# toposware/certificate-stark

Measured on AMD Instinct MI355X. Metric: proofs/sec, state_transition AIR @ 2^20 steps (complete prove(): trace gen, LDE, Blake3 commitments, constraint evaluation, composition, DEEP, FRI, 96 queries), higher is better.
Workload: dtype u64 (63-bit prime field, Montgomery) + u32 (Blake3)

## Files before the change

certificate-stark_amd/csrc/capi.hip:

```cpp
#include <hip/hip_runtime.h>
#include <stdio.h>
#include <stdlib.h>
#include <string.h>
#include <deque>
#include <new>
#include <vector>
#include "../../include/cstark.h"
#include "air_tx_host.h"
#include "blake3.h"
#include "ctx.h"
#include "constraints.h"
#include "deep.h"
#include "ext.h"
#include "generator_fold.h"
#include "hostfield.h"
#include "ntt.h"
#include "trace_gen.h"

namespace cs { thread_local char g_err[512] = ""; }
using cs::fail;
using cs::NttPlan;
using cs::CosetTable;
using cs::PeriodicTable;
using cs::g_err;
// ... 581 lines not shown
    HIP_TRY(hipSetDevice(c->device));
    const size_t N = (size_t)1 << (log_n + log_blowup);
    RC_TRY(ensure_ws(c, 2 * N * 8));
    uint64_t *nat = (uint64_t *)c->ws, *h = nat + N;
    if (log_blowup <= 3) {
        const NttPlan *pn, *pN;
        RC_TRY(get_plan(c, log_n, &pn));
        RC_TRY(get_plan(c, log_n + log_blowup, &pN));
        cs::NttArgs a{};
        a.in = d_combined; a.scratch = h; a.out = nat; a.width = 1u << log_blowup; a.batch = 1; a.log_n = log_n;
        a.w = pn->winv; a.post_scale = pn->n_inv; a.do_scale = true; a.inverse = true; a.aux = pn->aux_winv;
        HIP_TRY(cs::ntt_columns(a, c->stream));
        const uint64_t b_inv = cs::host::inv(cs::host::from_u64(1ull << log_blowup));
        HIP_TRY(cs::coset_combine(nat, h, log_n, log_blowup, pN->winv, b_inv, c->stream));
        HIP_TRY(cs::split_columns(h, d_cols, log_n, log_blowup, cs::host::inv(cs::host::lde_offset()), c->stream));
        return CSTARK_OK;
    }
    HIP_TRY(cs::interleave_cosets(d_combined, nat, log_n, log_blowup, c->stream));
    const NttPlan *p;
    RC_TRY(get_plan(c, log_n + log_blowup, &p));
    cs::NttArgs a{};
    a.in = nat; a.scratch = nat; a.out = h; a.width = 1; a.batch = 1; a.log_n = log_n + log_blowup;
    a.w = p->winv; a.post_scale = p->n_inv; a.do_scale = true; a.inverse = true; a.aux = p->aux_winv;
    HIP_TRY(cs::ntt_columns(a, c->stream));
    HIP_TRY(cs::split_columns(h, d_cols, log_n, log_blowup, cs::host::inv(cs::host::lde_offset()), c->stream));
    return CSTARK_OK;
}

int cstark_evaluate_polys_at(cstark_ctx *c, const uint64_t *d_coeffs, uint32_t width, uint32_t log_n, const uint64_t *points, uint32_t npts,
                             uint64_t *out ) {
    if (!c || !d_coeffs || !points || !out || width == 0 || npts == 0 || npts > 16) return fail(CSTARK_ERR_INVALID_ARG, "cstark_evaluate_polys_at: bad argument");
    if (log_n > 30) return fail(CSTARK_ERR_INVALID_ARG, "bad polynomial size");
    HIP_TRY(hipSetDevice(c->device));
    const size_t need = ((size_t)npts + (size_t)npts * width + cs::poly_eval_scratch_words(width, log_n, npts)) * 8;
    if (need > c->desc_bytes) {
        if (c->desc_buf) { HIP_TRY(hipStreamSynchronize(c->stream)); HIP_TRY(hipFree(c->desc_buf)); c->desc_buf = nullptr; c->desc_bytes = 0; }
        HIP_TRY(hipMalloc(&c->desc_buf, need));
        c->desc_bytes = need;
    }
    uint64_t *d_pts = (uint64_t *)c->desc_buf, *d_out = d_pts + npts, *d_scr = d_out + (size_t)npts * width;
    HIP_TRY(hipMemcpyAsync(d_pts, points, (size_t)npts * 8, hipMemcpyHostToDevice, c->stream));
    HIP_TRY(cs::poly_eval(d_coeffs, width, log_n, d_pts, npts, d_out, d_scr, c->stream));
    HIP_TRY(hipMemcpyAsync(out, d_out, (size_t)npts * width * 8, hipMemcpyDeviceToHost, c->stream));
    HIP_TRY(cs::stream_wait(c->stream));
    return CSTARK_OK;
}

int cstark_deep_composition(cstark_ctx *c, const uint64_t *d_trace_lde, const uint64_t *d_comp_lde, uint32_t width, uint32_t n_comp,
                            uint64_t z, const uint64_t *ood_trace, const uint64_t *ood_comp, const uint64_t *alpha, const uint64_t *beta,
                            const uint64_t *delta, uint64_t deg_a, uint64_t deg_b, uint64_t *d_out, uint32_t log_n, uint32_t log_blowup,
                            uint32_t k0, uint32_t nk) {
    if (!c || !d_trace_lde || !d_comp_lde || !ood_trace || !ood_comp || !alpha || !beta || !delta || !d_out || nk == 0 || width == 0 || n_comp == 0)
        return fail(CSTARK_ERR_INVALID_ARG, "cstark_deep_composition: bad argument");
    if (log_n < cs::NTT_MIN_LOG_N || log_n > cs::NTT_MAX_LOG_N || log_blowup > 6 || (uint64_t)k0 + nk > (1ull << log_blowup)) return fail(CSTARK_ERR_INVALID_ARG, "bad domain parameters");
    HIP_TRY(hipSetDevice(c->device));
    const NttPlan *plan;
    RC_TRY(get_plan(c, log_n, &plan));
    const size_t b = (size_t)1 << log_blowup, nco = 2 * (size_t)width + n_comp, words = 2 * nco + b;
    if (c->deep_words < words) {
        HIP_TRY(hipStreamSynchronize(c->stream));
        if (c->deep_buf) { HIP_TRY(hipFree(c->deep_buf)); c->deep_buf = nullptr; }
        if (c->deep_stage) { HIP_TRY(hipHostFree(c->deep_stage)); c->deep_stage = nullptr; }
        c->deep_words = 0;
        HIP_TRY(hipMalloc((void **)&c->deep_buf, words * 8));
        HIP_TRY(hipHostMalloc((void **)&c->deep_stage, words * 8, hipHostMallocDefault));
        if (!c->deep_ev) HIP_TRY(hipEventCreateWithFlags(&c->deep_ev, hipEventDisableTiming));
        c->deep_words = words;
    } else {
        HIP_TRY(hipEventSynchronize(c->deep_ev));
    }
    uint64_t *blk = c->deep_stage;
    memcpy(blk, alpha, width * 8); memcpy(blk + width, beta, width * 8); memcpy(blk + 2 * width, delta, n_comp * 8);
    memcpy(blk + nco, ood_trace, 2 * (size_t)width * 8); memcpy(blk + nco + 2 * width, ood_comp, n_comp * 8);
    const uint64_t wbn = cs::host::root_of_unity(log_n + log_blowup);
    uint64_t shift = cs::host::lde_offset();
    for (size_t k = 0; k < b; k++) { blk[2 * nco + k] = shift; shift = cs::host::mul(shift, wbn); }
    HIP_TRY(hipMemcpyAsync(c->deep_buf, blk, words * 8, hipMemcpyHostToDevice, c->stream));
    HIP_TRY(hipEventRecord(c->deep_ev, c->stream));
    const uint64_t *d = c->deep_buf;
    cs::DeepParams p{};
    p.trace_lde = d_trace_lde; p.comp_lde = d_comp_lde; p.w = plan->w; p.coef = d; p.ood = d + nco; p.shifts = d + 2 * nco; p.out = d_out;
    p.z = z; p.zw = cs::host::mul(z, cs::host::root_of_unity(log_n)); p.zb = cs::host::pow(z, n_comp);
    p.deg_a = deg_a; p.deg_b = deg_b; p.width = width; p.nb = n_comp; p.log_n = log_n; p.k0 = k0;
    HIP_TRY(cs::deep_composition(p, nk, c->stream));
    return CSTARK_OK;
}

int cstark_interleave_cosets(cstark_ctx *c, const uint64_t *d_coset_major, uint64_t *d_natural, uint32_t log_n, uint32_t log_blowup) {
    if (!c || !d_coset_major || !d_natural || d_coset_major == d_natural) return fail(CSTARK_ERR_INVALID_ARG, "cstark_interleave_cosets: bad argument");
    if (log_n + log_blowup > 30 || log_blowup > 6) return fail(CSTARK_ERR_INVALID_ARG, "bad domain parameters");
    HIP_TRY(hipSetDevice(c->device));
    HIP_TRY(cs::interleave_cosets(d_coset_major, d_natural, log_n, log_blowup, c->stream));
    return CSTARK_OK;
}
int cstark_fri_fold4(cstark_ctx *c, const uint64_t *d_evals, uint64_t *d_out, uint32_t log_n, uint64_t domain_offset, uint64_t alpha) {
    if (!c || !d_evals || !d_out || d_evals == d_out) return fail(CSTARK_ERR_INVALID_ARG, "cstark_fri_fold4: bad argument");
    if (log_n < cs::NTT_MIN_LOG_N || log_n > cs::NTT_MAX_LOG_N) return fail(CSTARK_ERR_UNSUPPORTED, "layer size must be 2^6 .. 2^24");
    if (domain_offset == 0 || domain_offset >= cs::host::P || alpha >= cs::host::P) return fail(CSTARK_ERR_INVALID_ARG, "offset / alpha must be field elements");
    HIP_TRY(hipSetDevice(c->device));
    const NttPlan *p;
    RC_TRY(get_plan(c, log_n, &p));
    HIP_TRY(cs::fri_fold4(d_evals, d_out, log_n, p->winv, cs::host::inv(domain_offset), alpha, cs::host::inv(cs::host::from_u64(4)), c->stream));
    return CSTARK_OK;
}
int cstark_fri_fold(cstark_ctx *c, const uint64_t *d_evals, uint64_t *d_out, uint32_t log_n, uint32_t folding_factor, uint64_t domain_offset, uint64_t alpha) {
    if (!c || !d_evals || !d_out || d_evals == d_out) return fail(CSTARK_ERR_INVALID_ARG, "cstark_fri_fold: bad argument");
    if (folding_factor != 4 && folding_factor != 8 && folding_factor != 16) return fail(CSTARK_ERR_UNSUPPORTED, "FRI folding factor must be 4, 8 or 16");
    if (log_n < cs::NTT_MIN_LOG_N || log_n > cs::NTT_MAX_LOG_N) return fail(CSTARK_ERR_UNSUPPORTED, "layer size must be 2^6 .. 2^24");
    if (domain_offset == 0 || domain_offset >= cs::host::P || alpha >= cs::host::P) return fail(CSTARK_ERR_INVALID_ARG, "offset / alpha must be field elements");
    HIP_TRY(hipSetDevice(c->device));
    const NttPlan *p;
    RC_TRY(get_plan(c, log_n, &p));
    const unsigned log_f = folding_factor == 4 ? 2 : folding_factor == 8 ? 3 : 4;
    HIP_TRY(cs::fri_fold(d_evals, d_out, log_n, log_f, p->winv, cs::host::inv(domain_offset), alpha, cs::host::inv(cs::host::from_u64(folding_factor)), c->stream));
    return CSTARK_OK;
}

int cstark_evaluate_polys_at_ext(cstark_ctx *c, const uint64_t *d_coeffs, uint32_t width, uint32_t log_n, uint32_t m, const uint64_t *z, uint64_t *out) {
    if (!c || !d_coeffs || !z || !out || width == 0 || (m != 2 && m != 3)) return fail(CSTARK_ERR_INVALID_ARG, "cstark_evaluate_polys_at_ext: bad argument");
    if (log_n > 30) return fail(CSTARK_ERR_INVALID_ARG, "bad polynomial size");
    for (uint32_t i = 0; i < m; i++) if (z[i] >= cs::host::P) return fail(CSTARK_ERR_INVALID_ARG, "the point is not an extension element");
    HIP_TRY(hipSetDevice(c->device));
    const size_t need = ((size_t)m * width + cs::poly_eval_ext_scratch_words(width, log_n, m)) * 8;
    if (need > c->desc_bytes) {
        if (c->desc_buf) { HIP_TRY(hipStreamSynchronize(c->stream)); HIP_TRY(hipFree(c->desc_buf)); c->desc_buf = nullptr; c->desc_bytes = 0; }
        HIP_TRY(hipMalloc(&c->desc_buf, need));
        c->desc_bytes = need;
    }
    uint64_t *d_out = (uint64_t *)c->desc_buf, *d_scr = d_out + (size_t)m * width;
    HIP_TRY(cs::poly_eval_ext(d_coeffs, width, log_n, z, m, d_out, d_scr, c->stream));
    HIP_TRY(hipMemcpyAsync(out, d_out, (size_t)m * width * 8, hipMemcpyDeviceToHost, c->stream));
    HIP_TRY(cs::stream_wait(c->stream));
    return CSTARK_OK;
}
}

int fri_coin_fold_dev(cstark_ctx *c, uint32_t *d_seed, const uint8_t *d_root, uint64_t *d_alpha, uint32_t *d_root_out, const uint64_t *d_evals,
                      uint64_t *d_out, uint32_t log_n, uint32_t log_f, uint64_t domain_offset, uint32_t m) {
    if (log_n < cs::NTT_MIN_LOG_N || log_n > cs::NTT_MAX_LOG_N) return fail(CSTARK_ERR_UNSUPPORTED, "layer size must be 2^6 .. 2^24");
    if (m < 1 || m > 3) return fail(CSTARK_ERR_INVALID_ARG, "fri_coin_fold_dev: bad extension degree");
    const NttPlan *p;
    RC_TRY(get_plan(c, log_n, &p));
    const uint64_t offset_inv = cs::host::inv(domain_offset), inv_f = cs::host::inv(cs::host::from_u64(1ull << log_f));
    if (m == 1) {
        HIP_TRY(cs::fri_coin(d_seed, d_root, d_alpha, d_root_out, c->stream));
        HIP_TRY(cs::fri_fold(d_evals, d_out, log_n, log_f, p->winv, offset_inv, 0, inv_f, c->stream, d_alpha));
    } else {
        HIP_TRY(cs::fri_coin_ext(d_seed, d_root, d_alpha, d_root_out, m, c->stream));
        HIP_TRY(cs::fri_fold_ext(d_evals, d_out, log_n, log_f, p->winv, offset_inv, nullptr, m, inv_f, c->stream, d_alpha));
    }
    return CSTARK_OK;
}
int hash_rows_slots(cstark_ctx *c, uint32_t hash_fn, const uint64_t *d_lde, uint8_t *d_leaves, uint32_t width, uint32_t log_n, uint32_t log_blowup, uint32_t log_s) {
    if (!c || !d_lde || !d_leaves || width == 0 || width > 128 || hash_fn > 1 || log_blowup > 6 || log_s > log_blowup || ((uintptr_t)d_leaves & 15) != 0)
        return fail(CSTARK_ERR_INVALID_ARG, "hash_rows_slots: bad argument");
    HIP_TRY(hipSetDevice(c->device));
    if (hash_fn == 1) HIP_TRY(cs::hash_rows_sha3(d_lde, d_leaves, width, log_n, log_blowup, 0, 1u << log_blowup, c->stream, log_s));
    else HIP_TRY(cs::hash_rows(d_lde, d_leaves, width, log_n, log_blowup, 0, 1u << log_blowup, c->stream, log_s));
    return CSTARK_OK;
}
int evaluate_ood_frames(cstark_ctx *c, const uint64_t *d_coeffs, uint32_t width, const uint64_t *d_ccoef, uint32_t n_comp, uint32_t log_n,
                        const uint64_t zpts[2], uint64_t zb, uint64_t *out_trace, uint64_t *out_comp) {
    if (!c || !d_coeffs || !d_ccoef || !out_trace || !out_comp || width == 0 || n_comp == 0) return fail(CSTARK_ERR_INVALID_ARG, "evaluate_ood_frames: bad argument");
    HIP_TRY(hipSetDevice(c->device));
    const size_t n_out = 2 * (size_t)width + n_comp;
    const size_t scr_t = cs::poly_eval_scratch_words(width, log_n, 2), scr_c = cs::poly_eval_scratch_words(n_comp, log_n, 1);
// ... 1015 lines not shown
```

certificate-stark_amd/csrc/debug/debug_ood.hip:

```cpp
#include <hip/hip_runtime.h>
#include "../../../include/cstark_debug_ood.h"
#include "../ctx.h"
#include "../deep.h"
#include "../ntt.h"

extern "C" int cstark_debug_ood_deep_dev(void *ctx, uint32_t m, const uint64_t *d_pts, const uint64_t *d_coeffs, uint32_t width, const uint64_t *d_ccoef,
                                         uint32_t n_comp, const uint64_t *d_trace_lde, const uint64_t *d_comp_lde, const uint64_t *d_coef,
                                         const uint64_t *d_deg, const uint64_t *d_shifts, const uint64_t *d_ood_in, uint64_t *d_scal, uint32_t nk,
                                         uint32_t log_n, uint32_t log_blowup, uint64_t *d_frame, uint64_t *d_sums) {
    cstark_ctx *c = (cstark_ctx *)ctx;
    if (!c || !d_pts || !d_coeffs || !d_ccoef || !d_trace_lde || !d_comp_lde || !d_coef || !d_deg || !d_shifts || !d_scal || !d_frame || !d_sums)
        return CSTARK_ERR_INVALID_ARG;
    if (m < 1 || m > 3 || width == 0 || n_comp == 0 || log_n < cs::NTT_MIN_LOG_N || log_n > cs::NTT_MAX_LOG_N || log_blowup > 6 || nk == 0 ||
        nk > (1u << log_blowup))
        return CSTARK_ERR_INVALID_ARG;
    if (hipSetDevice(c->device) != hipSuccess) return CSTARK_ERR_HIP;
    hipStream_t st = c->stream;
    RC_TRY(desc_reserve(c, ood_frames_dev_scratch_bytes(width, n_comp, log_n, m)));
    if (m == 1) RC_TRY(ood_frames_dev(c, d_coeffs, width, d_ccoef, n_comp, log_n, d_pts, d_frame));
    else RC_TRY(ood_frames_dev_ext(c, d_coeffs, width, d_ccoef, n_comp, log_n, m, d_pts, d_frame));
    if (hipMemcpyAsync(d_scal, d_pts, (size_t)3 * m * 8, hipMemcpyDeviceToDevice, st) != hipSuccess) return CSTARK_ERR_HIP;
    if (hipMemcpyAsync(d_scal + 3 * m, d_deg, (size_t)2 * m * 8, hipMemcpyDeviceToDevice, st) != hipSuccess) return CSTARK_ERR_HIP;
    const uint64_t *d_ood = d_ood_in ? d_ood_in : d_frame;
    if (m == 1) {
        const uint64_t *pw, *pwinv;
        RC_TRY(plan_tables(c, log_n, &pw, &pwinv));
        cs::DeepParams p{};
        p.trace_lde = d_trace_lde; p.comp_lde = d_comp_lde; p.w = pw; p.coef = d_coef; p.ood = d_ood; p.shifts = d_shifts; p.out = d_sums;
        p.width = width; p.nb = n_comp; p.log_n = log_n; p.k0 = 0; p.scal = d_scal;
        if (cs::deep_composition(p, nk, st) != hipSuccess) return CSTARK_ERR_HIP;
    } else {
        RC_TRY(deep_composition_ext_dev(c, d_trace_lde, d_comp_lde, width, n_comp, m, d_coef, d_ood, d_scal, d_shifts, d_sums, log_n, log_blowup, nk));
    }
    return hipStreamSynchronize(st) == hipSuccess ? CSTARK_OK : CSTARK_ERR_HIP;
}
```

certificate-stark_amd/csrc/deep.h:

```cpp
#pragma once
#include <hip/hip_runtime.h>
#include <stddef.h>
#include <stdint.h>

namespace cs {

struct DeepParams {
    const uint64_t *trace_lde, *comp_lde;
    const uint64_t *w, *shifts;
    const uint64_t *coef;
    const uint64_t *ood;
    uint64_t *out;
    uint64_t z, zw, zb, deg_a, deg_b;
    uint32_t width, nb, log_n, k0;
    const uint64_t *scal;
};

size_t poly_eval_scratch_words(unsigned width, unsigned log_n, unsigned npts);
hipError_t poly_eval(const uint64_t *d_coeffs, unsigned width, unsigned log_n, const uint64_t *d_points, unsigned npts, uint64_t *d_out,
                     uint64_t *d_scratch, hipStream_t stream);
hipError_t deep_composition(const DeepParams &p, unsigned nk, hipStream_t stream);
hipError_t fri_fold4(const uint64_t *d_evals, uint64_t *d_out, unsigned log_n, const uint64_t *d_winv, uint64_t offset_inv, uint64_t alpha,
                     uint64_t inv4, hipStream_t stream, const uint64_t *d_alpha = nullptr);
hipError_t fri_fold(const uint64_t *d_evals, uint64_t *d_out, unsigned log_n, unsigned log_f, const uint64_t *d_winv, uint64_t offset_inv, uint64_t alpha,
                    uint64_t inv_f, hipStream_t stream, const uint64_t *d_alpha = nullptr);

}
```

certificate-stark_amd/csrc/deep.hip:

```cpp
#include "deep.h"
#include "fp.cuh"

namespace cs {
namespace {

#ifndef CS_PE_SEG
#define CS_PE_SEG 16384
#endif
constexpr int PE_SEG = CS_PE_SEG, PE_MAXPTS = 2;
template <int NP>
__global__ __launch_bounds__(256) void k_poly_eval_partial(const fp *__restrict__ coeffs, size_t n, const fp *__restrict__ points, fp *__restrict__ partial,
                                                           unsigned width, unsigned seg_len) {
    __shared__ fp part[NP][256];
    const unsigned segs = gridDim.x, seg = blockIdx.x, col = blockIdx.y, t = threadIdx.x;
    const fp *c = coeffs + (size_t)col * n + (size_t)seg * seg_len;
    fp z[NP], z256[NP], acc[NP];
#pragma unroll
    for (int p = 0; p < NP; p++) { z[p] = points[p]; z256[p] = fp_pow(z[p], 256); acc[p] = 0; }
    const unsigned per = (seg_len + 255) / 256;
    for (unsigned k = per; k-- > 0;) {
        const fp v = k * 256 + t < seg_len ? c[(size_t)k * 256 + t] : 0;
#pragma unroll
        for (int p = 0; p < NP; p++) acc[p] = fp_add(fp_mul(acc[p], z256[p]), v);
    }
#pragma unroll
    for (int p = 0; p < NP; p++) part[p][t] = fp_mul(acc[p], fp_pow(z[p], (uint64_t)seg * seg_len + t));
    __syncthreads();
    for (int s = 128; s > 0; s >>= 1) {
        if ((int)t < s) {
#pragma unroll
            for (int p = 0; p < NP; p++) part[p][t] = fp_add(part[p][t], part[p][t + s]);
        }
        __syncthreads();
    }
    if (t < NP) partial[((size_t)t * width + col) * segs + seg] = part[t][0];
}
__global__ void k_poly_eval_sum(const fp *__restrict__ partial, fp *__restrict__ out, unsigned total, unsigned segs) {
    const unsigned i = blockIdx.x * blockDim.x + threadIdx.x;
    if (i >= total) return;
    fp a = 0;
    for (unsigned s = 0; s < segs; s++) a = fp_add(a, partial[(size_t)i * segs + s]);
    out[i] = a;
}

__global__ __launch_bounds__(256) void k_deep(DeepParams p) {
    const size_t n = (size_t)1 << p.log_n;
    const size_t j = blockIdx.x * (size_t)256 + threadIdx.x;
    if (j >= n) return;
    const unsigned kk = blockIdx.y;
    const fp x = fp_mul(p.shifts[p.k0 + kk], p.w[j]);
    const fp pz = p.scal ? p.scal[0] : p.z, pzw = p.scal ? p.scal[1] : p.zw, pzb = p.scal ? p.scal[2] : p.zb;
    const fp d1 = fp_sub(x, pz), d2 = fp_sub(x, pzw), d3 = fp_sub(x, pzb);
    const fp inv = fp_inv(fp_mul(fp_mul(d1, d2), d3));
    const fp i1 = fp_mul(inv, fp_mul(d2, d3)), i2 = fp_mul(inv, fp_mul(d1, d3)), i3 = fp_mul(inv, fp_mul(d1, d2));
    Acc128 s1 = acc_zero(), s2 = acc_zero(), s3 = acc_zero();
    const fp *t = p.trace_lde + (size_t)kk * p.width * n + j;
    for (unsigned c = 0; c < p.width; c++) {
        const fp v = t[(size_t)c * n];
        acc_mad(s1, p.coef[c], fp_sub(v, p.ood[c]));
        acc_mad(s2, p.coef[p.width + c], fp_sub(v, p.ood[p.width + c]));
        if ((c & 3) == 3) { acc_fold(s1); acc_fold(s2); }
    }
    acc_fold(s1); acc_fold(s2);
    const fp *h = p.comp_lde + (size_t)kk * p.nb * n + j;
    for (unsigned i = 0; i < p.nb; i++) {
        acc_mad(s3, p.coef[2 * p.width + i], fp_sub(h[(size_t)i * n], p.ood[2 * p.width + i]));
        if ((i & 3) == 3) acc_fold(s3);
    }
    acc_fold(s3);
    fp acc = fp_add(fp_add(fp_mul(acc_reduce(s1), i1), fp_mul(acc_reduce(s2), i2)), fp_mul(acc_reduce(s3), i3));
    const fp dga = p.scal ? p.scal[3] : p.deg_a, dgb = p.scal ? p.scal[4] : p.deg_b;
    p.out[(size_t)kk * n + j] = fp_mul(acc, fp_add(dga, fp_mul(dgb, x)));
}

__global__ __launch_bounds__(256) void k_fri_fold4(const fp *__restrict__ evals, fp *__restrict__ out, size_t q, const fp *__restrict__ winv,
                                                   fp offset_inv, fp alpha, fp inv4, const fp *__restrict__ alpha_dev) {
    const size_t i = blockIdx.x * (size_t)256 + threadIdx.x;
    if (i >= q) return;
    if (alpha_dev) alpha = *alpha_dev;
    const fp v0 = evals[i], v1 = evals[i + q], v2 = evals[i + 2 * q], v3 = evals[i + 3 * q];
    const fp zi = winv[q];
    const fp a = fp_add(v0, v2), b = fp_sub(v0, v2), c = fp_add(v1, v3), d = fp_mul(fp_sub(v1, v3), zi);
    const fp s0 = fp_add(a, c), s2 = fp_sub(a, c), s1 = fp_add(b, d), s3 = fp_sub(b, d);
    const fp r = fp_mul(alpha, fp_mul(offset_inv, winv[i]));
    const fp r2 = fp_sqr(r), r3 = fp_mul(r2, r);
    fp acc = fp_add(fp_add(s0, fp_mul(r, s1)), fp_add(fp_mul(r2, s2), fp_mul(r3, s3)));
    out[i] = fp_mul(acc, inv4);
}

template <int LOG_F>
__global__ __launch_bounds__(256) void k_fri_fold(const fp *__restrict__ evals, fp *__restrict__ out, size_t q, const fp *__restrict__ winv,
                                                  fp offset_inv, fp alpha, fp inv_f, const fp *__restrict__ alpha_dev) {
    constexpr int F = 1 << LOG_F;
    const size_t i = blockIdx.x * (size_t)256 + threadIdx.x;
    if (i >= q) return;
    if (alpha_dev) alpha = *alpha_dev;
    fp v[F];
#pragma unroll
    for (int t = 0; t < F; t++) v[t] = evals[i + (size_t)t * q];
#pragma unroll
    for (int len = F; len >= 2; len >>= 1) {
        const int half = len >> 1, step = F / len;
#pragma unroll
        for (int base = 0; base < F; base += len) {
#pragma unroll
            for (int t = 0; t < half; t++) {
                const fp a = v[base + t], b = v[base + t + half];
                v[base + t] = fp_add(a, b);
                const fp d = fp_sub(a, b);
                v[base + t + half] = (t == 0) ? d : fp_mul(d, winv[(size_t)(t * step) * q]);
            }
        }
    }
    const fp r = fp_mul(alpha, fp_mul(offset_inv, winv[i]));
    fp acc = 0;
#pragma unroll
    for (int k = F - 1; k >= 0; k--) {
        int br = 0;
#pragma unroll
        for (int bit = 0; bit < LOG_F; bit++) br |= ((k >> bit) & 1) << (LOG_F - 1 - bit);
        acc = fp_add(fp_mul(acc, r), v[br]);
    }
    out[i] = fp_mul(acc, inv_f);
}

}

hipError_t fri_fold4(const uint64_t *d_evals, uint64_t *d_out, unsigned log_n, const uint64_t *d_winv, uint64_t offset_inv, uint64_t alpha,
                     uint64_t inv4, hipStream_t stream, const uint64_t *d_alpha) {
    const size_t q = ((size_t)1 << log_n) / 4;
    hipLaunchKernelGGL(k_fri_fold4, dim3((unsigned)((q + 255) / 256)), dim3(256), 0, stream, d_evals, d_out, q, d_winv, offset_inv, alpha, inv4, d_alpha);
    return hipGetLastError();
}
hipError_t fri_fold(const uint64_t *d_evals, uint64_t *d_out, unsigned log_n, unsigned log_f, const uint64_t *d_winv, uint64_t offset_inv, uint64_t alpha,
                    uint64_t inv_f, hipStream_t stream, const uint64_t *d_alpha) {
    if (log_f == 2) return fri_fold4(d_evals, d_out, log_n, d_winv, offset_inv, alpha, inv_f, stream, d_alpha);
    if ((log_f != 3 && log_f != 4) || log_n < log_f) return hipErrorInvalidValue;
    const size_t q = ((size_t)1 << log_n) >> log_f;
    const dim3 grid((unsigned)((q + 255) / 256));
    if (log_f == 3) hipLaunchKernelGGL(k_fri_fold<3>, grid, dim3(256), 0, stream, d_evals, d_out, q, d_winv, offset_inv, alpha, inv_f, d_alpha);
    else hipLaunchKernelGGL(k_fri_fold<4>, grid, dim3(256), 0, stream, d_evals, d_out, q, d_winv, offset_inv, alpha, inv_f, d_alpha);
    return hipGetLastError();
}

size_t poly_eval_scratch_words(unsigned width, unsigned log_n, unsigned npts) {
    const size_t n = (size_t)1 << log_n, seg = n < (size_t)PE_SEG ? n : (size_t)PE_SEG;
    return (size_t)npts * width * (n / seg);
}
hipError_t poly_eval(const uint64_t *d_coeffs, unsigned width, unsigned log_n, const uint64_t *d_points, unsigned npts, uint64_t *d_out,
                     uint64_t *d_scratch, hipStream_t stream) {
    const size_t n = (size_t)1 << log_n;
    const unsigned seg_len = (unsigned)(n < (size_t)PE_SEG ? n : (size_t)PE_SEG), segs = (unsigned)(n / seg_len);
    for (unsigned p0 = 0; p0 < npts; p0 += PE_MAXPTS) {
        const unsigned np = npts - p0 >= 2 ? 2 : 1;
        fp *part = d_scratch + (size_t)p0 * width * segs;
        if (np == 2) hipLaunchKernelGGL(k_poly_eval_partial<2>, dim3(segs, width), dim3(256), 0, stream, d_coeffs, n, d_points + p0, part, width, seg_len);
        else hipLaunchKernelGGL(k_poly_eval_partial<1>, dim3(segs, width), dim3(256), 0, stream, d_coeffs, n, d_points + p0, part, width, seg_len);
    }
    const unsigned total = npts * width;
    hipLaunchKernelGGL(k_poly_eval_sum, dim3((total + 255) / 256), dim3(256), 0, stream, d_scratch, d_out, total, segs);
    return hipGetLastError();
}
hipError_t deep_composition(const DeepParams &p, unsigned nk, hipStream_t stream) {
    const size_t n = (size_t)1 << p.log_n;
    hipLaunchKernelGGL(k_deep, dim3((unsigned)((n + 255) / 256), nk), dim3(256), 0, stream, p);
    return hipGetLastError();
}

}
```

certificate-stark_amd/csrc/prove.hip:

```cpp
#include <hip/hip_runtime.h>
#include <string.h>
#include <algorithm>
#include <atomic>
#include <new>
#include <chrono>
#include <thread>
#include <vector>
#include "../../include/cstark.h"
#include "ctx.h"
#include "blake3.h"
#include "channel.h"
#include "deep.h"
#include "ext.h"
#include "range_batch.h"
#include "hostblake3.h"
#include "keccak.cuh"
#include "air_tx_host.h"
#include "hostfield.h"
#include "coin.h"
#include "proof_layout.h"
#include "transcript.h"

namespace cs {

// ... 715 lines not shown
    RC_TRY(arena_extra(c, a, 43, &d_chan, 12 * m * 8 + n_ood * 8));
    if (m == 1) {
        RC_TRY(arena_extra(c, a, 41, &d_fri, (size_t)(8 + 10 * 32) * 4));
        RC_TRY(arena_extra(c, a, 40, &dcoef, n * 8));
        sums = R.deep;
    } else {
        RC_TRY(arena_extra(c, a, 47, &d_fri, (size_t)(8 + 2 * 3 * 32) * 4));
        RC_TRY(arena_extra(c, a, 48, &sums, 3 * n * 8));
        RC_TRY(arena_extra(c, a, 49, &dcoef, 3 * n * 8));
    }
    uint64_t *d_pts = d_chan, *d_scal = d_chan + 4 * m, *d_deepc = d_chan + 12 * m, *d_ood = (uint64_t *)(d_res + o_ood);
    uint32_t *d_cnt = (uint32_t *)(d_res + o_cnt);
    RC_TRY(host_open_block(a, off));
    RC_TRY(desc_reserve(c, ood_frames_dev_scratch_bytes((uint32_t)W, (uint32_t)ce, log_n, m)));
    uint64_t *d_coef_block;
    const bool is_tx = job.air == CSTARK_AIR_STATE_TRANSITION;
    const size_t coef_stride = is_tx ? (size_t)CE_COEF_WORDS : 230 + 2 * (size_t)job.n_assertions;
    if (is_tx) RC_TRY(tx_coef_device_block(c, &d_coef_block));
    else RC_TRY(arena_extra(c, a, 46, &d_coef_block, m * coef_stride * 8));
    const uint64_t *pw, *pwinv;
    RC_TRY(plan_tables(c, log_n, &pw, &pwinv));

    RC_TRY(commit_trace_leaves(c, a, R));
    RC_TRY(cstark_merkle_build_fn(c, R.opt.hash_fn, a->tnodes, log_N));
    STAGE();
    {
        ChanStep s{};
        s.seed = d_fri; s.m = m;
        const std::vector<uint8_t> prefix = channel_seed(job.width, log_n, *opt, log_b, R.log_rem);
        if (job.air == CSTARK_AIR_SCHNORR) {
            uint8_t key[12] = {};
            memcpy(key, prefix.data(), 2); memcpy(key + 2, prefix.data() + 10, 7); key[11] = 1;
            if (memcmp(key, c->schnorr_seed_key, sizeof key) != 0) {
                const std::vector<uint8_t> seed = channel_seed(job, *opt, R.log_rem);
                hostb3::hash(seed.data(), seed.size(), c->schnorr_seed);
                memcpy(c->schnorr_seed_key, key, sizeof key);
            }
            HIP_TRY(hipMemcpyAsync(d_fri, c->schnorr_seed, 32, hipMemcpyHostToDevice, st));
        } else {
            s.init = 1; s.pub = a->d_pub; s.npub = job.air == CSTARK_AIR_RANGE ? 1 : 14;
        }
        memcpy(s.prefix, prefix.data(), SEED_PREFIX); s.prefix_len = SEED_PREFIX;
        s.absorb[0].kind = CHAN_DIGEST; s.absorb[0].ptr = a->tnodes + 32; s.absorb[0].copy_out = d_res + o_troot;
        s.draw = CHAN_DRAW_COEFFS; s.a = job.n_constraints; s.b = job.n_assertions; s.stride = CSTARK_TX_NUM_CONSTRAINTS;
        s.set_stride = (uint32_t)coef_stride;
        s.count = (uint32_t)transcript::coefficient_draws(job.n_constraints, job.n_assertions); s.out = d_coef_block;
        HIP_TRY(channel_step(s, st));
    }
    if (is_tx) {
        RC_TRY(tx_evaluate_constraints_sets(c, a->lde, nullptr, m, nullptr, R.comb, job.item, log_n, 3, 0, 8, true, a->d_pub));
    } else {
        job.d_avalues = job.air == CSTARK_AIR_RANGE ? a->d_pub + 1 : job.air == CSTARK_AIR_SCHNORR ? nullptr : a->d_pub;
        for (unsigned q = 0; q < m; q++) {
            job.d_coefs = d_coef_block + q * coef_stride;
            RC_TRY(job.combine(c, a, job, nullptr, nullptr, nullptr, nullptr, R.comb[q]));
        }
    }
    STAGE();
    RC_TRY(commit_composition(c, a, R));
    STAGE();
    {
        ChanStep s{};
        s.seed = d_fri; s.m = m;
        s.absorb[0].kind = CHAN_DIGEST; s.absorb[0].ptr = a->cnodes + 32; s.absorb[0].copy_out = d_res + o_croot;
        s.draw = CHAN_DRAW_POINT; s.count = 1; s.b = (uint32_t)ce; s.w = host::root_of_unity(log_n); s.out = d_pts; s.out2 = d_scal;
        HIP_TRY(channel_step(s, st));
    }
    if (m == 1) RC_TRY(ood_frames_dev(c, a->coeffs, (uint32_t)W, R.ccoefs, (uint32_t)ce, log_n, d_pts, d_ood));
    else RC_TRY(ood_frames_dev_ext(c, a->coeffs, (uint32_t)W, R.ccoefs, (uint32_t)ce, log_n, m, d_pts, d_ood));
    STAGE();
    {
        ChanStep s{};
        s.seed = d_fri; s.m = m;
        s.absorb[0].kind = CHAN_ELEMS; s.absorb[0].ptr = d_ood; s.absorb[0].count = (uint32_t)(2 * m * W);
        s.absorb[1].kind = CHAN_ELEMS; s.absorb[1].ptr = d_ood + 2 * m * W; s.absorb[1].count = (uint32_t)(m * ce);
        s.draw = CHAN_DRAW_DEEP; s.a = (uint32_t)W; s.b = (uint32_t)ce; s.per = CSTARK_CONV_DEEP_DRAWS_PER_REGISTER;
        s.count = (uint32_t)transcript::deep_draws(W, ce); s.out = d_deepc; s.out2 = d_scal;
        HIP_TRY(channel_step(s, st));
    }
    if (m == 1) {
        cs::DeepParams p{};
        p.trace_lde = a->lde; p.comp_lde = R.clde; p.w = pw; p.coef = d_deepc; p.ood = d_ood; p.shifts = a->d_shifts; p.out = sums;
        p.width = (uint32_t)W; p.nb = (uint32_t)ce; p.log_n = log_n; p.k0 = 0; p.scal = d_scal;
        HIP_TRY(cs::deep_composition(p, 1, st));
    } else {
        RC_TRY(deep_composition_ext_dev(c, a->lde, R.clde, (uint32_t)W, (uint32_t)ce, m, d_deepc, d_ood, d_scal, a->d_shifts, sums, log_n, log_b, 1));
    }
    RC_TRY(deep_extend(c, R, sums, dcoef));
    const hipEvent_t deep_done = a->ev[R.evi];
    STAGE();
    RC_TRY(fri_commit(c, a, R, d_fri, (uint32_t *)(d_res + o_lroots), (uint64_t *)(d_res + o_remainder)));
    STAGE();
    {
        ChanStep s{};
        s.seed = d_fri; s.m = m;
        s.absorb[0].kind = CHAN_ELEMS; s.absorb[0].ptr = d_res + o_remainder; s.absorb[0].count = (uint32_t)rem_len; s.absorb[0].copy_out = d_res + o_rem;
        s.absorb[1].kind = CHAN_INT; s.absorb[1].value = 1;
        s.draw = CHAN_DRAW_QUERIES; s.count = (uint32_t)nq; s.log_domain = log_N; s.log_f = R.log_f; s.n_layers = n_layers; s.slot = 256;
        s.pos = a->d_pos; s.cnt = d_cnt;
        HIP_TRY(channel_step(s, st));
    }
    RC_TRY(open_stage(c, a, S, {R.clde, R.layer.data(), R.log_s(), nullptr, d_cnt + 1, nullptr, 0}, d_res, O));
    STAGE();
    static const bool hostprof = getenv("CSTARK_HOSTPROF") != nullptr;
    const auto hp1 = std::chrono::steady_clock::now();
    HIP_TRY(cs::stream_wait_tail(st, deep_done));
    const auto hp2 = std::chrono::steady_clock::now();
    a->timed = true; a->channel = CSTARK_CHANNEL_DEVICE;
    const uint8_t *h = a->h_open;
    const uint32_t *cnt = (const uint32_t *)(h + o_cnt);
    if (cnt[0] != nq) return fail(CSTARK_ERR_HIP, "device channel: the query positions could not be drawn");
    for (unsigned l = 0; l < n_layers; l++)
        if (cnt[l + 1] == 0 || cnt[l + 1] > nq) return fail(CSTARK_ERR_HIP, "device channel: bad folded position count");
    ProofParts p{};
    p.trace_root = h + o_troot; p.cons_root = h + o_croot; p.layer_roots = h + o_lroots; p.rem_commit = h + o_rem;
    p.ood_trace = h + o_ood; p.ood_comp = h + o_ood + ood_trace_bytes(S); p.remainder = h + o_remainder;
    p.nonce = 1;
    RC_TRY(finish_proof(S, p, h, O, cnt + 1, proof, capacity, proof_len));
    if (hostprof) {
        const auto hp3 = std::chrono::steady_clock::now();
        auto us = [](auto d) { return std::chrono::duration<double, std::micro>(d).count(); };
        fprintf(stderr, "[cstark hostprof] device channel: enqueued in %.0f us, waited %.0f us, proof written in %.0f us\n", us(hp1 - hp0), us(hp2 - hp1), us(hp3 - hp2));
    }
    return CSTARK_OK;
}
#undef STAGE
bool use_dev_channel(const cstark_options *opt, const AirJob &job) {
    static const bool host_env = [] { const char *e = getenv("CSTARK_HOST_CHANNEL"); return e && atoi(e) != 0; }();
    if (host_env || job.sharded || job.n_constraints > CSTARK_TX_NUM_CONSTRAINTS) return false;
    if (opt->hash_fn != 0 || opt->field_extension > 2 || opt->grinding_factor != 0) return false;
    uint32_t lb = 0, lf = 0, lr = 0;
    while ((1u << lb) < opt->blowup_factor && lb < 8) lb++;
    while ((1u << lf) < opt->fri_folding_factor && lf < 8) lf++;
    while ((1u << lr) < opt->fri_max_remainder && lr < 12) lr++;
    return lf >= 2 && job.log_n + lb > lr;
}

bool shard_split(uint32_t nk) {
    static const bool on = [] { const char *e = getenv("CSTARK_SHARD_SPLIT"); return !e || atoi(e) != 0; }();
    return on && (nk == 2 || nk == 4);
}
uint32_t shard_rows(uint32_t nk) { return shard_split(nk) ? nk / 2 + 4 : nk; }

int gather_roots(cstark_ctx *c, ProveArena *a, AirJob &job, uint32_t reg0 = 58) {
    const size_t n = (size_t)1 << job.log_n;
    k_gather_pub<<<1, 64, 0, c->stream>>>(a->trace, n, a->d_pub, reg0);
    HIP_TRY(hipGetLastError());
    if (job.dev_channel) return CSTARK_OK;
    job.pub.assign(14, 0);
    HIP_TRY(hipMemcpyAsync(job.pub.data(), a->d_pub, 14 * 8, hipMemcpyDeviceToHost, c->stream));
    return CSTARK_OK;
}


int tx_build(cstark_ctx *c, ProveArena *a, AirJob &job) {
    static const int mode = [] { const char *e = getenv("CSTARK_TRACE_OVERLAP"); return e ? atoi(e) : 1; }();
    if (mode == 0) {
        RC_TRY(cstark_tx_build_trace(c, a->trace));
        return gather_roots(c, a, job);
    }
    RC_TRY(tx_build_trace_split(c, a->trace));
    if (mode == 2) {
        for (hipEvent_t e : {c->ev_join, c->ev_mid, c->ev_join2}) HIP_TRY(hipStreamWaitEvent(c->stream, e, 0));
        return gather_roots(c, a, job);
    }
    const size_t n = (size_t)1 << job.log_n;
// ... 623 lines not shown
```

Baseline: 42.14.

## Factor OOD constants out of DEEP loop, batch inversions, table-driven poly eval

Result: no change. 42.47, median of 6 (+0.8%).

```diff
diff --git a/certificate-stark_amd/csrc/capi.hip b/certificate-stark_amd/csrc/capi.hip
--- a/certificate-stark_amd/csrc/capi.hip
+++ b/certificate-stark_amd/csrc/capi.hip
@@ -687,6 +687,11 @@
     p.trace_lde = d_trace_lde; p.comp_lde = d_comp_lde; p.w = plan->w; p.coef = d; p.ood = d + nco; p.shifts = d + 2 * nco; p.out = d_out;
     p.z = z; p.zw = cs::host::mul(z, cs::host::root_of_unity(log_n)); p.zb = cs::host::pow(z, n_comp);
     p.deg_a = deg_a; p.deg_b = deg_b; p.width = width; p.nb = n_comp; p.log_n = log_n; p.k0 = k0;
+    for (uint32_t e = 0; e < width; e++) {
+        p.k1 = cs::host::add(p.k1, cs::host::mul(alpha[e], ood_trace[e]));
+        p.k2 = cs::host::add(p.k2, cs::host::mul(beta[e], ood_trace[width + e]));
+    }
+    for (uint32_t e = 0; e < n_comp; e++) p.k3 = cs::host::add(p.k3, cs::host::mul(delta[e], ood_comp[e]));
     HIP_TRY(cs::deep_composition(p, nk, c->stream));
     return CSTARK_OK;
 }
diff --git a/certificate-stark_amd/csrc/debug/debug_ood.hip b/certificate-stark_amd/csrc/debug/debug_ood.hip
--- a/certificate-stark_amd/csrc/debug/debug_ood.hip
+++ b/certificate-stark_amd/csrc/debug/debug_ood.hip
@@ -28,6 +28,7 @@
         cs::DeepParams p{};
         p.trace_lde = d_trace_lde; p.comp_lde = d_comp_lde; p.w = pw; p.coef = d_coef; p.ood = d_ood; p.shifts = d_shifts; p.out = d_sums;
         p.width = width; p.nb = n_comp; p.log_n = log_n; p.k0 = 0; p.scal = d_scal;
+        if (cs::deep_consts(d_coef, d_ood, d_scal, width, n_comp, st) != hipSuccess) return CSTARK_ERR_HIP;
         if (cs::deep_composition(p, nk, st) != hipSuccess) return CSTARK_ERR_HIP;
     } else {
         RC_TRY(deep_composition_ext_dev(c, d_trace_lde, d_comp_lde, width, n_comp, m, d_coef, d_ood, d_scal, d_shifts, d_sums, log_n, log_blowup, nk));
diff --git a/certificate-stark_amd/csrc/deep.h b/certificate-stark_amd/csrc/deep.h
--- a/certificate-stark_amd/csrc/deep.h
+++ b/certificate-stark_amd/csrc/deep.h
@@ -12,6 +12,7 @@
     const uint64_t *ood;
     uint64_t *out;
     uint64_t z, zw, zb, deg_a, deg_b;
+    uint64_t k1, k2, k3;
     uint32_t width, nb, log_n, k0;
     const uint64_t *scal;
 };
@@ -19,6 +20,7 @@
 size_t poly_eval_scratch_words(unsigned width, unsigned log_n, unsigned npts);
 hipError_t poly_eval(const uint64_t *d_coeffs, unsigned width, unsigned log_n, const uint64_t *d_points, unsigned npts, uint64_t *d_out,
                      uint64_t *d_scratch, hipStream_t stream);
+hipError_t deep_consts(const uint64_t *d_coef, const uint64_t *d_ood, uint64_t *d_scal, unsigned width, unsigned n_comp, hipStream_t stream);
 hipError_t deep_composition(const DeepParams &p, unsigned nk, hipStream_t stream);
 hipError_t fri_fold4(const uint64_t *d_evals, uint64_t *d_out, unsigned log_n, const uint64_t *d_winv, uint64_t offset_inv, uint64_t alpha,
                      uint64_t inv4, hipStream_t stream, const uint64_t *d_alpha = nullptr);
diff --git a/certificate-stark_amd/csrc/deep.hip b/certificate-stark_amd/csrc/deep.hip
--- a/certificate-stark_amd/csrc/deep.hip
+++ b/certificate-stark_amd/csrc/deep.hip
@@ -7,24 +7,58 @@
 #ifndef CS_PE_SEG
 #define CS_PE_SEG 16384
 #endif
-constexpr int PE_SEG = CS_PE_SEG, PE_MAXPTS = 2;
+constexpr int PE_SEG = CS_PE_SEG, PE_MAXPTS = 2, PE_FOLD = 4;
+__host__ __device__ inline size_t pe_table_words(size_t nk) { return 256 + nk; }
+__global__ __launch_bounds__(256) void k_pe_tables(const fp *__restrict__ points, fp *__restrict__ tab, unsigned nk) {
+    const unsigned i = blockIdx.x * 256 + threadIdx.x;
+    if (i >= 256 + nk) return;
+    tab[blockIdx.y * pe_table_words(nk) + i] = fp_pow(points[blockIdx.y], i < 256 ? (uint64_t)i : (uint64_t)(i - 256) * 256);
+}
 template <int NP>
-__global__ __launch_bounds__(256) void k_poly_eval_partial(const fp *__restrict__ coeffs, size_t n, const fp *__restrict__ points, fp *__restrict__ partial,
-                                                           unsigned width, unsigned seg_len) {
+__global__ __launch_bounds__(256) void k_poly_eval_partial(const fp *__restrict__ coeffs, size_t n, const fp *__restrict__ tab, fp *__restrict__ partial,
+                                                           unsigned width, unsigned seg_len, unsigned nk) {
     __shared__ fp part[NP][256];
     const unsigned segs = gridDim.x, seg = blockIdx.x, col = blockIdx.y, t = threadIdx.x;
     const fp *c = coeffs + (size_t)col * n + (size_t)seg * seg_len;
-    fp z[NP], z256[NP], acc[NP];
-#pragma unroll
-    for (int p = 0; p < NP; p++) { z[p] = points[p]; z256[p] = fp_pow(z[p], 256); acc[p] = 0; }
     const unsigned per = (seg_len + 255) / 256;
-    for (unsigned k = per; k-- > 0;) {
+    const fp *zk = tab + 256 + (size_t)seg * per;
+    Acc128 acc[NP];
+#pragma unroll
+    for (int p = 0; p < NP; p++) acc[p] = acc_zero();
+    const auto block = [&](const fp (&v)[PE_FOLD], unsigned k) {
+#pragma unroll
+        for (int u = 0; u < PE_FOLD; u++) {
+#pragma unroll
+            for (int p = 0; p < NP; p++) acc_mad(acc[p], zk[p * pe_table_words(nk) + k + u], v[u]);
+        }
+#pragma unroll
+        for (int p = 0; p < NP; p++) acc_fold(acc[p]);
+    };
+    const unsigned whole = per - per % PE_FOLD;
+    if (whole) {
+        fp v[PE_FOLD];
+#pragma unroll
+        for (int u = 0; u < PE_FOLD; u++) v[u] = c[(size_t)u * 256 + t];
+        for (unsigned k = PE_FOLD; k < whole; k += PE_FOLD) {
+            fp next[PE_FOLD];
+#pragma unroll
+            for (int u = 0; u < PE_FOLD; u++) next[u] = c[(size_t)(k + u) * 256 + t];
+            block(v, k - PE_FOLD);
+#pragma unroll
+            for (int u = 0; u < PE_FOLD; u++) v[u] = next[u];
+        }
+        block(v, whole - PE_FOLD);
+    }
+    for (unsigned k = whole; k < per; k++) {
         const fp v = k * 256 + t < seg_len ? c[(size_t)k * 256 + t] : 0;
 #pragma unroll
-        for (int p = 0; p < NP; p++) acc[p] = fp_add(fp_mul(acc[p], z256[p]), v);
-    }
-#pragma unroll
-    for (int p = 0; p < NP; p++) part[p][t] = fp_mul(acc[p], fp_pow(z[p], (uint64_t)seg * seg_len + t));
+        for (int p = 0; p < NP; p++) acc_mad(acc[p], zk[p * pe_table_words(nk) + k], v);
+    }
+#pragma unroll
+    for (int p = 0; p < NP; p++) {
+        acc_fold(acc[p]);
+        part[p][t] = fp_mul(acc_reduce(acc[p]), tab[p * pe_table_words(nk) + t]);
+    }
     __syncthreads();
     for (int s = 128; s > 0; s >>= 1) {
         if ((int)t < s) {
@@ -43,34 +77,94 @@
     out[i] = a;
 }
 
+__global__ __launch_bounds__(256) void k_deep_consts(const fp *__restrict__ coef, const fp *__restrict__ ood, fp *__restrict__ scal, unsigned width, unsigned nb) {
+    __shared__ fp part[3][256];
+    const unsigned t = threadIdx.x;
+    const unsigned first[4] = {0, width, 2 * width, 2 * width + nb};
+#pragma unroll
+    for (int w = 0; w < 3; w++) {
+        fp k = 0;
+        for (unsigned e = first[w] + t; e < first[w + 1]; e += 256) k = fp_add(k, fp_mul(coef[e], ood[e]));
+        part[w][t] = k;
+    }
+    __syncthreads();
+    for (int s = 128; s > 0; s >>= 1) {
+        if ((int)t < s)
+            for (int w = 0; w < 3; w++) part[w][t] = fp_add(part[w][t], part[w][t + s]);
+        __syncthreads();
+    }
+    if (t < 3) scal[5 + t] = part[t][0];
+}
+
+#ifndef CS_DEEP_P
+#define CS_DEEP_P 4
+#endif
+template <int P>
 __global__ __launch_bounds__(256) void k_deep(DeepParams p) {
-    const size_t n = (size_t)1 << p.log_n;
+    const size_t n = (size_t)1 << p.log_n, q = n / P;
     const size_t j = blockIdx.x * (size_t)256 + threadIdx.x;
-    if (j >= n) return;
+    if (j >= q) return;
     const unsigned kk = blockIdx.y;
-    const fp x = fp_mul(p.shifts[p.k0 + kk], p.w[j]);
-    const fp pz = p.scal ? p.scal[0] : p.z, pzw = p.scal ? p.scal[1] : p.zw, pzb = p.scal ? p.scal[2] : p.zb;
-    const fp d1 = fp_sub(x, pz), d2 = fp_sub(x, pzw), d3 = fp_sub(x, pzb);
-    const fp inv = fp_inv(fp_mul(fp_mul(d1, d2), d3));
-    const fp i1 = fp_mul(inv, fp_mul(d2, d3)), i2 = fp_mul(inv, fp_mul(d1, d3)), i3 = fp_mul(inv, fp_mul(d1, d2));
-    Acc128 s1 = acc_zero(), s2 = acc_zero(), s3 = acc_zero();
+    Acc128 s1[P], s2[P];
+#pragma unroll
+    for (int i = 0; i < P; i++) { s1[i] = acc_zero(); s2[i] = acc_zero(); }
     const fp *t = p.trace_lde + (size_t)kk * p.width * n + j;
     for (unsigned c = 0; c < p.width; c++) {
-        const fp v = t[(size_t)c * n];
-        acc_mad(s1, p.coef[c], fp_sub(v, p.ood[c]));
-        acc_mad(s2, p.coef[p.width + c], fp_sub(v, p.ood[p.width + c]));
-        if ((c & 3) == 3) { acc_fold(s1); acc_fold(s2); }
-    }
-    acc_fold(s1); acc_fold(s2);
+        const fp a = p.coef[c], b = p.coef[p.width + c];
+#pragma unroll
+        for (int i = 0; i < P; i++) {
+            const fp v = t[(size_t)c * n + i * q];
+            acc_mad(s1[i], a, v);
+            acc_mad(s2[i], b, v);
+        }
+        if ((c & 3) == 3) {
+#pragma unroll
+            for (int i = 0; i < P; i++) { acc_fold(s1[i]); acc_fold(s2[i]); }
+        }
+    }
+    const fp k1 = p.scal ? p.scal[5] : p.k1, k2 = p.scal ? p.scal[6] : p.k2, k3 = p.scal ? p.scal[7] : p.k3;
+    fp e1[P], e2[P], e3[P];
+#pragma unroll
+    for (int i = 0; i < P; i++) {
+        acc_fold(s1[i]); acc_fold(s2[i]);
+        e1[i] = fp_sub(acc_reduce(s1[i]), k1);
+        e2[i] = fp_sub(acc_reduce(s2[i]), k2);
+        s1[i] = acc_zero();
+    }
     const fp *h = p.comp_lde + (size_t)kk * p.nb * n + j;
-    for (unsigned i = 0; i < p.nb; i++) {
-        acc_mad(s3, p.coef[2 * p.width + i], fp_sub(h[(size_t)i * n], p.ood[2 * p.width + i]));
-        if ((i & 3) == 3) acc_fold(s3);
-    }
-    acc_fold(s3);
-    fp acc = fp_add(fp_add(fp_mul(acc_reduce(s1), i1), fp_mul(acc_reduce(s2), i2)), fp_mul(acc_reduce(s3), i3));
+    for (unsigned c = 0; c < p.nb; c++) {
+        const fp d = p.coef[2 * p.width + c];
+#pragma unroll
+        for (int i = 0; i < P; i++) acc_mad(s1[i], d, h[(size_t)c * n + i * q]);
+        if ((c & 3) == 3) {
+#pragma unroll
+            for (int i = 0; i < P; i++) acc_fold(s1[i]);
+        }
+    }
+#pragma unroll
+    for (int i = 0; i < P; i++) { acc_fold(s1[i]); e3[i] = fp_sub(acc_reduce(s1[i]), k3); }
+    const fp pz = p.scal ? p.scal[0] : p.z, pzw = p.scal ? p.scal[1] : p.zw, pzb = p.scal ? p.scal[2] : p.zb;
     const fp dga = p.scal ? p.scal[3] : p.deg_a, dgb = p.scal ? p.scal[4] : p.deg_b;
-    p.out[(size_t)kk * n + j] = fp_mul(acc, fp_add(dga, fp_mul(dgb, x)));
+    const fp shift = p.shifts[p.k0 + kk];
+    fp num[P], den[P], pre[P];
+#pragma unroll
+    for (int i = 0; i < P; i++) {
+        const fp x = fp_mul(shift, p.w[j + i * q]);
+        const fp d1 = fp_sub(x, pz), d2 = fp_sub(x, pzw), d3 = fp_sub(x, pzb);
+        const fp d12 = fp_mul(d1, d2), d13 = fp_mul(d1, d3), d23 = fp_mul(d2, d3);
+        Acc128 a = acc_zero();
+        acc_mad(a, e1[i], d23); acc_mad(a, e2[i], d13); acc_mad(a, e3[i], d12);
+        num[i] = fp_mul(acc_reduce(a), fp_add(dga, fp_mul(dgb, x)));
+        den[i] = fp_mul(d12, d3);
+        pre[i] = i ? fp_mul(pre[i ? i - 1 : 0], den[i]) : den[i];
+    }
+    fp inv = fp_inv(pre[P - 1]);
+#pragma unroll
+    for (int i = P - 1; i > 0; i--) {
+        p.out[(size_t)kk * n + j + i * q] = fp_mul(num[i], fp_mul(inv, pre[i - 1]));
+        inv = fp_mul(inv, den[i]);
+    }
+    p.out[(size_t)kk * n + j] = fp_mul(num[0], inv);
 }
 
 __global__ __launch_bounds__(256) void k_fri_fold4(const fp *__restrict__ evals, fp *__restrict__ out, size_t q, const fp *__restrict__ winv,
@@ -144,27 +238,36 @@
 }
 
 size_t poly_eval_scratch_words(unsigned width, unsigned log_n, unsigned npts) {
-    const size_t n = (size_t)1 << log_n, seg = n < (size_t)PE_SEG ? n : (size_t)PE_SEG;
-    return (size_t)npts * width * (n / seg);
+    const size_t n = (size_t)1 << log_n, seg = n < (size_t)PE_SEG ? n : (size_t)PE_SEG, nk = n < 256 ? 1 : n / 256;
+    return (size_t)npts * width * (n / seg) + (size_t)npts * pe_table_words(nk);
 }
 hipError_t poly_eval(const uint64_t *d_coeffs, unsigned width, unsigned log_n, const uint64_t *d_points, unsigned npts, uint64_t *d_out,
                      uint64_t *d_scratch, hipStream_t stream) {
     const size_t n = (size_t)1 << log_n;
     const unsigned seg_len = (unsigned)(n < (size_t)PE_SEG ? n : (size_t)PE_SEG), segs = (unsigned)(n / seg_len);
+    const unsigned nk = (unsigned)(n < 256 ? 1 : n / 256);
+    fp *tab = d_scratch + (size_t)npts * width * segs;
+    hipLaunchKernelGGL(k_pe_tables, dim3((unsigned)((pe_table_words(nk) + 255) / 256), npts), dim3(256), 0, stream, d_points, tab, nk);
     for (unsigned p0 = 0; p0 < npts; p0 += PE_MAXPTS) {
         const unsigned np = npts - p0 >= 2 ? 2 : 1;
         fp *part = d_scratch + (size_t)p0 * width * segs;
-        if (np == 2) hipLaunchKernelGGL(k_poly_eval_partial<2>, dim3(segs, width), dim3(256), 0, stream, d_coeffs, n, d_points + p0, part, width, seg_len);
-        else hipLaunchKernelGGL(k_poly_eval_partial<1>, dim3(segs, width), dim3(256), 0, stream, d_coeffs, n, d_points + p0, part, width, seg_len);
+        const fp *tp = tab + (size_t)p0 * pe_table_words(nk);
+        if (np == 2) hipLaunchKernelGGL(k_poly_eval_partial<2>, dim3(segs, width), dim3(256), 0, stream, d_coeffs, n, tp, part, width, seg_len, nk);
+        else hipLaunchKernelGGL(k_poly_eval_partial<1>, dim3(segs, width), dim3(256), 0, stream, d_coeffs, n, tp, part, width, seg_len, nk);
     }
     const unsigned total = npts * width;
     hipLaunchKernelGGL(k_poly_eval_sum, dim3((total + 255) / 256), dim3(256), 0, stream, d_scratch, d_out, total, segs);
     return hipGetLastError();
 }
+hipError_t deep_consts(const uint64_t *d_coef, const uint64_t *d_ood, uint64_t *d_scal, unsigned width, unsigned n_comp, hipStream_t stream) {
+    hipLaunchKernelGGL(k_deep_consts, dim3(1), dim3(256), 0, stream, d_coef, d_ood, d_scal, width, n_comp);
+    return hipGetLastError();
+}
 hipError_t deep_composition(const DeepParams &p, unsigned nk, hipStream_t stream) {
-    const size_t n = (size_t)1 << p.log_n;
-    hipLaunchKernelGGL(k_deep, dim3((unsigned)((n + 255) / 256), nk), dim3(256), 0, stream, p);
-    return hipGetLastError();
-}
-
-}
+    const size_t n = (size_t)1 << p.log_n, q = n / CS_DEEP_P;
+    if (q == 0) return hipErrorInvalidValue;
+    hipLaunchKernelGGL(k_deep<CS_DEEP_P>, dim3((unsigned)((q + 255) / 256), nk), dim3(256), 0, stream, p);
+    return hipGetLastError();
+}
+
+}
diff --git a/certificate-stark_amd/csrc/prove.hip b/certificate-stark_amd/csrc/prove.hip
--- a/certificate-stark_amd/csrc/prove.hip
+++ b/certificate-stark_amd/csrc/prove.hip
@@ -821,6 +821,7 @@
         cs::DeepParams p{};
         p.trace_lde = a->lde; p.comp_lde = R.clde; p.w = pw; p.coef = d_deepc; p.ood = d_ood; p.shifts = a->d_shifts; p.out = sums;
         p.width = (uint32_t)W; p.nb = (uint32_t)ce; p.log_n = log_n; p.k0 = 0; p.scal = d_scal;
+        HIP_TRY(cs::deep_consts(d_deepc, d_ood, d_scal, (uint32_t)W, (uint32_t)ce, st));
         HIP_TRY(cs::deep_composition(p, 1, st));
     } else {
         RC_TRY(deep_composition_ext_dev(c, a->lde, R.clde, (uint32_t)W, (uint32_t)ce, m, d_deepc, d_ood, d_scal, a->d_shifts, sums, log_n, log_b, 1));
```
